# sp-uhh/audio-visual-vad

Measured on AMD Instinct MI355X. Metric: AV frame-pairs/sec (fwd+bwd), higher is better.
Workload: dtype f32; 1 GPU; AV_net fused training step (WaveNet-W0 encoder + ResNet-18 trunk + concat + 2xLSTM1024 + FC, masked BCE, backward, RCCL all-reduce, fused Adam): BASELINE configs[3]/[4] per-GPU shard; per_gpu_frame_pairs=1024, global_frame_pairs=1024, sequences_per_gpu=64, parallelism=dp1, reserved_cus=0, reported_block=median

## Files before the change

audio-visual-vad_amd/csrc/bn_kernels.h:

```cpp
#pragma once
#include "common.h"

constexpr int BN_MAXC = 1024;
constexpr int MAXC = BN_MAXC;
constexpr int STAT_CHUNKS = 512;

template <int MODE>
__global__ void __launch_bounds__(256)
    col_reduce(const float* __restrict__ x, const float* __restrict__ dy, const float* __restrict__ ymask,
               const float* __restrict__ mean, const float* __restrict__ invstd, long M, int C, long rows_per_chunk,
               double* __restrict__ part, const float* __restrict__ msc = nullptr, const float* __restrict__ msh = nullptr,
               const unsigned char* __restrict__ qmask = nullptr) {
  __shared__ double sm[256 * 8];
  const int t = threadIdx.x;
  const int Q = C >> 2, RL = 256 / Q;
  const int q = t % Q, rl = t / Q;
  double s[4] = {0, 0, 0, 0}, ss[4] = {0, 0, 0, 0};
  float mu[4] = {0, 0, 0, 0}, is[4] = {1, 1, 1, 1};
  float ksc[4] = {0, 0, 0, 0}, ksh[4] = {0, 0, 0, 0};
  if (MODE == 1) {
#pragma unroll
    for (int j = 0; j < 4; ++j) { mu[j] = mean[q * 4 + j]; is[j] = invstd[q * 4 + j]; }
    if (msc) {
#pragma unroll
// ... 90 lines not shown
  const int c = blockIdx.x * FIN_CH + (threadIdx.x % FIN_CH);
  if (c >= C || threadIdx.x >= FIN_CH) return;
  float mean, var;
  if (training) {
    const double m = s / (double)M;
    double v = ss / (double)M - m * m;
    if (v < 0) v = 0;
    mean = (float)m; var = (float)v;
    const double unb = M > 1 ? v * (double)M / (double)(M - 1) : v;
    rm[c] = (1.f - momentum) * rm[c] + momentum * mean;
    rv[c] = (1.f - momentum) * rv[c] + momentum * (float)unb;
  } else {
    mean = rm[c]; var = rv[c];
  }
  const float is = 1.0f / sqrtf(var + eps);
  const float sc = gamma[c] * is;
  scale[c] = sc;
  shift[c] = beta[c] - mean * sc;
  mean_o[c] = mean;
  invstd_o[c] = is;
}

__global__ void bn_bwd_finalize(const double* __restrict__ part, int nchunk, long M, int C, const float* __restrict__ gamma,
                                const float* __restrict__ invstd, int training, float* __restrict__ dgamma,
                                float* __restrict__ dbeta, float* __restrict__ coef) {
  double s = 0, ss = 0;
  chunk_sums(part, nchunk, C, s, ss);
  const int c = blockIdx.x * FIN_CH + (threadIdx.x % FIN_CH);
  if (c >= C || threadIdx.x >= FIN_CH) return;
  if (dbeta) dbeta[c] += (float)s;
  if (dgamma) dgamma[c] += (float)ss;
  coef[c] = gamma[c] * invstd[c];
  coef[MAXC + c] = training ? (float)(s / (double)M) : 0.f;
  coef[2 * MAXC + c] = training ? (float)(ss / (double)M) : 0.f;
}

__device__ __forceinline__ float bn_affine(float x, float sc, float sh) { return fmaf(x, sc, sh); }

typedef __bf16 bn_bf16x4 __attribute__((ext_vector_type(4)));
typedef float bn_f32x4 __attribute__((ext_vector_type(4)));
__device__ __forceinline__ void store_quad_bf16(void* base, long quad, const float (&o)[4]) {
  const bn_f32x4 f = {o[0], o[1], o[2], o[3]};
  reinterpret_cast<bn_bf16x4*>(base)[quad] = __builtin_convertvector(f, bn_bf16x4);
}
__device__ __forceinline__ float4 load_quad_bf16(const void* base, long quad) {
  const bn_bf16x4 h = reinterpret_cast<const bn_bf16x4*>(base)[quad];
  const bn_f32x4 f = __builtin_convertvector(h, bn_f32x4);
  return make_float4(f[0], f[1], f[2], f[3]);
}

__device__ __forceinline__ float4 ld4(const float* p, int c) { return *reinterpret_cast<const float4*>(p + c); }

template <bool OB = false, bool IB = false>
__global__ void __launch_bounds__(256)
    bn_act(const float* __restrict__ x, const float* __restrict__ scale, const float* __restrict__ shift,
           const float* __restrict__ idn, const float* __restrict__ iscale, const float* __restrict__ ishift,
           float* __restrict__ y, long nquad, int C, int relu, unsigned char* __restrict__ qmask_out = nullptr) {
  const bool fixed = (256 % (C >> 2)) == 0;
  long i = (long)blockIdx.x * blockDim.x + threadIdx.x;
  int c = (int)((i * 4) % C);
  float4 sc = ld4(scale, c), sh = ld4(shift, c), a = make_float4(0, 0, 0, 0), b = a;
  if (iscale) { a = ld4(iscale, c); b = ld4(ishift, c); }
  for (; i < nquad; i += (long)gridDim.x * blockDim.x) {
    if (!fixed) {
      c = (int)((i * 4) % C);
      sc = ld4(scale, c); sh = ld4(shift, c);
      if (iscale) { a = ld4(iscale, c); b = ld4(ishift, c); }
    }
    const float4 v = reinterpret_cast<const float4*>(x)[i];
    float o[4] = {bn_affine(v.x, sc.x, sh.x), bn_affine(v.y, sc.y, sh.y), bn_affine(v.z, sc.z, sh.z), bn_affine(v.w, sc.w, sh.w)};
    if (idn) {
      const float4 d = IB ? load_quad_bf16(idn, i) : reinterpret_cast<const float4*>(idn)[i];
      if (iscale) {
        o[0] += bn_affine(d.x, a.x, b.x); o[1] += bn_affine(d.y, a.y, b.y);
        o[2] += bn_affine(d.z, a.z, b.z); o[3] += bn_affine(d.w, a.w, b.w);
      } else { o[0] += d.x; o[1] += d.y; o[2] += d.z; o[3] += d.w; }
    }
    if (relu) { o[0] = fmaxf(o[0], 0.f); o[1] = fmaxf(o[1], 0.f); o[2] = fmaxf(o[2], 0.f); o[3] = fmaxf(o[3], 0.f); }
    if constexpr (OB) store_quad_bf16(y, i, o);
    else reinterpret_cast<float4*>(y)[i] = make_float4(o[0], o[1], o[2], o[3]);
    if (qmask_out)
      qmask_out[i] = (unsigned char)((o[0] > 0.f ? 1 : 0) | (o[1] > 0.f ? 2 : 0) | (o[2] > 0.f ? 4 : 0) | (o[3] > 0.f ? 8 : 0));
  }
}

template <bool OB = false>
__global__ void __launch_bounds__(256)
    bn_bwd_apply(const float* __restrict__ x, const float* dy, const float* __restrict__ ymask,
                 const float* __restrict__ mean, const float* __restrict__ invstd, const float* __restrict__ coef,
                 float* dx, float* gout, long nquad, int C, const float* __restrict__ msc = nullptr,
                 const float* __restrict__ msh = nullptr, const unsigned char* __restrict__ qmask = nullptr) {
  const bool fixed = (256 % (C >> 2)) == 0;
  long i = (long)blockIdx.x * blockDim.x + threadIdx.x;
  int c = (int)((i * 4) % C);
  float4 mu = ld4(mean, c), is = ld4(invstd, c), k0 = ld4(coef, c), k1 = ld4(coef + MAXC, c), k2 = ld4(coef + 2 * MAXC, c);
  float4 ms = make_float4(0, 0, 0, 0), mh = ms;
  if (msc) { ms = ld4(msc, c); mh = ld4(msh, c); }
  for (; i < nquad; i += (long)gridDim.x * blockDim.x) {
    if (!fixed) {
      c = (int)((i * 4) % C);
      mu = ld4(mean, c); is = ld4(invstd, c); k0 = ld4(coef, c); k1 = ld4(coef + MAXC, c); k2 = ld4(coef + 2 * MAXC, c);
      if (msc) { ms = ld4(msc, c); mh = ld4(msh, c); }
    }
    const float4 xv = reinterpret_cast<const float4*>(x)[i];
    const float4 d = reinterpret_cast<const float4*>(dy)[i];
    float g[4] = {d.x, d.y, d.z, d.w};
    if (ymask) {
      const float4 y = reinterpret_cast<const float4*>(ymask)[i];
      if (!(y.x > 0.f)) g[0] = 0.f;
      if (!(y.y > 0.f)) g[1] = 0.f;
      if (!(y.z > 0.f)) g[2] = 0.f;
      if (!(y.w > 0.f)) g[3] = 0.f;
    } else if (qmask) {
      const unsigned qm = qmask[i];
      if (!(qm & 1u)) g[0] = 0.f;
      if (!(qm & 2u)) g[1] = 0.f;
      if (!(qm & 4u)) g[2] = 0.f;
      if (!(qm & 8u)) g[3] = 0.f;
    } else if (msc) {
      if (!(fmaf(xv.x, ms.x, mh.x) > 0.f)) g[0] = 0.f;
      if (!(fmaf(xv.y, ms.y, mh.y) > 0.f)) g[1] = 0.f;
      if (!(fmaf(xv.z, ms.z, mh.z) > 0.f)) g[2] = 0.f;
      if (!(fmaf(xv.w, ms.w, mh.w) > 0.f)) g[3] = 0.f;
    }
    const float xs[4] = {xv.x, xv.y, xv.z, xv.w};
    const float m4[4] = {mu.x, mu.y, mu.z, mu.w}, i4[4] = {is.x, is.y, is.z, is.w};
    const float a4[4] = {k0.x, k0.y, k0.z, k0.w}, b4[4] = {k1.x, k1.y, k1.z, k1.w}, c4[4] = {k2.x, k2.y, k2.z, k2.w};
    float o[4];
#pragma unroll
    for (int j = 0; j < 4; ++j) {
      const float xh = (xs[j] - m4[j]) * i4[j];
      o[j] = a4[j] * (g[j] - b4[j] - xh * c4[j]);
    }
    if constexpr (OB) store_quad_bf16(dx, i, o);
    else reinterpret_cast<float4*>(dx)[i] = make_float4(o[0], o[1], o[2], o[3]);
    if (gout) reinterpret_cast<float4*>(gout)[i] = make_float4(g[0], g[1], g[2], g[3]);
  }
}
```

audio-visual-vad_amd/csrc/trunk.hip:

```cpp
#include "bgemm.h"
#include "conv64.h"

using convop::Geom;

namespace {

#include "bn_kernels.h"

constexpr int NCONV = AVVAD_TRUNK_NCONV;

constexpr int NBLOCK = 8;
constexpr int WIDTHS[4] = {64, 128, 256, 512};

struct Block {
  int stage, width;
  int h, w;
  long M;
  bool ds;
  int i1, i2, id;
  size_t in;
  size_t c1, a1;
  size_t c2, cd;
  size_t out, qm;
};
// ... 287 lines not shown
__global__ void __launch_bounds__(256)
    stem_pool_relu_bwd(const float* __restrict__ c0, const float* __restrict__ scale, const float* __restrict__ shift,
                       const unsigned* __restrict__ am, const float* __restrict__ dp0, float* __restrict__ g0,
                       int N, int Hc, int Wc, int Hp, int Wp, const float* __restrict__ mean = nullptr,
                       const float* __restrict__ invstd = nullptr, double* __restrict__ part = nullptr) {
  __shared__ double sm[256 * 8];
  const long total = (long)N * Hc * Wc * 16;
  float s4[4] = {0.f, 0.f, 0.f, 0.f}, q4[4] = {0.f, 0.f, 0.f, 0.f};
  float mu[4] = {0.f, 0.f, 0.f, 0.f}, is[4] = {1.f, 1.f, 1.f, 1.f};
  if (part) {
    const int qc = (int)(((long)blockIdx.x * blockDim.x + threadIdx.x) & 15);
#pragma unroll
    for (int k = 0; k < 4; ++k) { mu[k] = mean[qc * 4 + k]; is[k] = invstd[qc * 4 + k]; }
  }
  for (long i = (long)blockIdx.x * blockDim.x + threadIdx.x; i < total; i += (long)gridDim.x * blockDim.x) {
    const int q = (int)(i & 15);
    long r = i >> 4;
    const int w = (int)(r % Wc); r /= Wc;
    const int h = (int)(r % Hc); const int n = (int)(r / Hc);
    const float4 sc = *reinterpret_cast<const float4*>(scale + q * 4), sh = *reinterpret_cast<const float4*>(shift + q * 4);
    const float4 v = reinterpret_cast<const float4*>(c0)[i];
    const bool pos[4] = {bn_affine(v.x, sc.x, sh.x) > 0.f, bn_affine(v.y, sc.y, sh.y) > 0.f, bn_affine(v.z, sc.z, sh.z) > 0.f,
                         bn_affine(v.w, sc.w, sh.w) > 0.f};
    float g[4] = {0, 0, 0, 0};
    const int ph0 = max(0, h / 2), ph1 = min(Hp - 1, (h + 1) / 2);
    const int pw0 = max(0, w / 2), pw1 = min(Wp - 1, (w + 1) / 2);
    for (int ph = ph0; ph <= ph1; ++ph)
      for (int pw = pw0; pw <= pw1; ++pw) {
        if (h < 2 * ph - 1 || h > 2 * ph + 1 || w < 2 * pw - 1 || w > 2 * pw + 1) continue;
        const unsigned me = (unsigned)((h - (2 * ph - 1)) * 3 + (w - (2 * pw - 1)));
        const long o = ((long)(n * Hp + ph) * Wp + pw) * 16 + q;
        const unsigned a = am[o];
        const float4 dp = reinterpret_cast<const float4*>(dp0)[o];
        if (pos[0] && (a & 255u) == me) g[0] += dp.x;
        if (pos[1] && ((a >> 8) & 255u) == me) g[1] += dp.y;
        if (pos[2] && ((a >> 16) & 255u) == me) g[2] += dp.z;
        if (pos[3] && (a >> 24) == me) g[3] += dp.w;
      }
    reinterpret_cast<float4*>(g0)[i] = make_float4(g[0], g[1], g[2], g[3]);
    if (part) {
      const float xv[4] = {v.x, v.y, v.z, v.w};
#pragma unroll
      for (int k = 0; k < 4; ++k) { s4[k] += g[k]; q4[k] = fmaf(g[k], (xv[k] - mu[k]) * is[k], q4[k]); }
    }
  }
  if (part == nullptr) return;
#pragma unroll
  for (int k = 0; k < 4; ++k) { sm[threadIdx.x * 8 + k] = (double)s4[k]; sm[threadIdx.x * 8 + 4 + k] = (double)q4[k]; }
  __syncthreads();
  if (threadIdx.x < 64) {
    const int c = threadIdx.x, cq = c >> 2, cj = c & 3;
    double a = 0, b = 0;
    for (int l = 0; l < 16; ++l) { a += sm[(l * 16 + cq) * 8 + cj]; b += sm[(l * 16 + cq) * 8 + 4 + cj]; }
    part[((long)blockIdx.x * 2 + 0) * 64 + c] = a;
    part[((long)blockIdx.x * 2 + 1) * 64 + c] = b;
  }
}

template <bool IB = false>
__global__ void avgpool_fwd(const float* __restrict__ y, float* __restrict__ feat, int N, int HW, int C) {
  const long total = (long)N * C;
  for (long i = (long)blockIdx.x * blockDim.x + threadIdx.x; i < total; i += (long)gridDim.x * blockDim.x) {
    const int c = (int)(i % C); const long n = i / C;
    float s = 0.f;
    for (int p = 0; p < HW; ++p) s += IB ? (float)reinterpret_cast<const __bf16*>(y)[(n * HW + p) * C + c] : y[(n * HW + p) * C + c];
    feat[i] = s / (float)HW;
  }
}
__global__ void avgpool_bwd(const float* __restrict__ dfeat, float* __restrict__ dy, int N, int HW, int C) {
  const long total = (long)N * HW * C;
  const float inv = 1.f / (float)HW;
  for (long i = (long)blockIdx.x * blockDim.x + threadIdx.x; i < total; i += (long)gridDim.x * blockDim.x) {
    const int c = (int)(i % C); const long n = i / ((long)HW * C);
    dy[i] = dfeat[n * C + c] * inv;
  }
}
__global__ void zero_f32(float* p, long n) {
  for (long i = (long)blockIdx.x * blockDim.x + threadIdx.x; i < n; i += (long)gridDim.x * blockDim.x) p[i] = 0.f;
}

static inline int ew_grid(long n) { long b = (n + 255) / 256; return (int)(b > 4096 ? 4096 : (b < 1 ? 1 : b)); }

constexpr int STEM_WH = 17;
__global__ void __launch_bounds__(256)
    stem_wgrad_mfma(const float* __restrict__ x, const float* __restrict__ dy, float* __restrict__ slab, int N, int H, int W,
                    int Ho, int Wo, int LDW) {
  extern __shared__ float img[];
  const int lane = threadIdx.x & 63, wave = threadIdx.x >> 6;
  const int li = lane & 31, lh = lane >> 5;
  const int mt = wave >> 1, nt = wave & 1;
  const int tap = mt * 32 + li;
  const int tc = tap < 49 ? tap : 0;
  const int abase = (tc / 7) * LDW + (tc % 7) + 2 * lh;
  const int PH = H + 6, wh = Wo >> 1;
  for (int i = threadIdx.x; i < PH * LDW; i += 256) img[i] = 0.f;
  f32x16 acc;
#pragma unroll
  for (int r = 0; r < 16; ++r) acc[r] = 0.f;
  const int voff = (lh * 64 + nt * 32 + li) * 4;
  for (int n = blockIdx.x; n < N; n += gridDim.x) {
    __syncthreads();
    const float* xn = x + (long)n * H * W;
    for (int i = threadIdx.x; i < H * W; i += 256) {
      const int r = i / W, c = i - r * W;
      img[(r + 3) * LDW + c + 3] = xn[i];
    }
    __syncthreads();
    const __amdgpu_buffer_rsrc_t rdy = brsrc(dy + (long)n * Ho * Wo * 64, Ho * Wo * 64 * 4);
    constexpr int RB = 4;
    float b0[RB][STEM_WH], b1[RB][STEM_WH];
    auto rowload = [&](int ho0, float (&b)[RB][STEM_WH]) {
#pragma unroll
      for (int rr = 0; rr < RB; ++rr)
#pragma unroll
        for (int sw = 0; sw < STEM_WH; ++sw)
          b[rr][sw] = bload(rdy, (sw < wh && ho0 + rr < Ho) ? voff : BUF_OOB, ((ho0 + rr) * Wo + 2 * sw) * 256);
    };
    auto rowmul = [&](int ho0, const float (&b)[RB][STEM_WH]) {
#pragma unroll
      for (int rr = 0; rr < RB; ++rr) {
        if (ho0 + rr >= Ho) break;
        const float* ap = img + abase + 2 * (ho0 + rr) * LDW;
#pragma unroll
        for (int sw = 0; sw < STEM_WH; ++sw)
          if (sw < wh) acc = mfma32(ap[4 * sw], b[rr][sw], acc);
      }
    };
    rowload(0, b0);
    for (int ho = 0; ho < Ho; ho += 2 * RB) {
      if (ho + RB < Ho) rowload(ho + RB, b1);
      __builtin_amdgcn_sched_barrier(0);
      rowmul(ho, b0);
      if (ho + RB >= Ho) break;
      if (ho + 2 * RB < Ho) rowload(ho + 2 * RB, b0);
      __builtin_amdgcn_sched_barrier(0);
      rowmul(ho + RB, b1);
    }
  }
  float* out = slab + (long)blockIdx.x * (49 * 64);
#pragma unroll
  for (int r = 0; r < 16; ++r) {
    const int t = mt * 32 + mfma32_row(r, lh);
    if (t < 49) out[t * 64 + nt * 32 + li] = acc[r];
  }
}
__global__ void __launch_bounds__(256) stem_wgrad_reduce(const float* __restrict__ slab, int nslab, float* __restrict__ pk) {
  __shared__ float sm[8][32];
  const int el = threadIdx.x & 31, grp = threadIdx.x >> 5;
  const int i = blockIdx.x * 32 + el;
  float s = 0.f;
#pragma unroll 4
  for (int b = grp; b < nslab; b += 8) s += slab[(long)b * (49 * 64) + i];
  sm[grp][el] = s;
  __syncthreads();
  if (grp != 0) return;
#pragma unroll
  for (int k = 1; k < 8; ++k) s += sm[k][el];
  pk[i] = s;
}

static inline bool fits_u30(long n) { return n >= 0 && n < (1L << 30); }
static inline bool taps_fit(const Geom& g) { return g.KS * g.KS <= 32; }
static inline bool fits_buf(long n_floats) { return n_floats >= 0 && n_floats < (1L << 29) - 64; }
static inline bool stem_kernel_ok(const Geom& g) {
  const int LDW = (g.W + 6) | 1;
  return g.C == 1 && g.KS == 7 && g.stride == 2 && g.pad == 3 && g.Co == 64 && (size_t)(g.H + 6) * LDW * sizeof(float) <= 48 * 1024 &&
         !avvad_tune().no_stem_kernel;
}
static inline bool stem_wgrad_ok(const Geom& g, bool slab) {
  return stem_kernel_ok(g) && (g.Wo & 1) == 0 && g.Wo <= 2 * STEM_WH && slab && (long)g.Ho * g.Wo * 64 * 4 < (1L << 31);
}
static inline long cls_tile_cap() {
  if (avvad_tune().cls_cap > 0) return avvad_tune().cls_cap;
  return 4L * grid_cus();
}
static inline bool cls_common(const Geom& g, bool slab) {
  return avvad_tune().bf16 == 0 && !avvad_tune().no_cls && slab && g.KS == 3 && g.pad == 1 && g.N >= 128 && g.C % 32 == 0 &&
         g.Co % 32 == 0 && g.Ho >= 2 && g.Wo >= 2 && avvad_tune().igemm_variant < 0 && !avvad_tune().no_buf &&
         avvad_tune().no_streamk == 0;
}
static inline bool conv_fwd_cls_ok(const Geom& g, bool slab) {
  if (!cls_common(g, slab) || g.Co % 4 || g.Co < 128) return false;
  const long tiles = (long)g.Ho * g.Wo * cdiv(g.N, 128) * cdiv(g.Co, 128);
  return tiles <= cls_tile_cap() &&
         fits_buf((long)g.N * g.H * g.W * g.C) && fits_buf(9L * g.C * g.Co);
}
static inline bool conv_dgrad_cls_ok(const Geom& g, bool slab) {
  if (!cls_common(g, slab) || (g.stride != 1 && (g.stride != 2 || avvad_tune().no_s2_cls)) || g.C % 4 || g.C < 128) return false;
  const long tiles = (long)g.H * g.W * cdiv(g.N, 128) * cdiv(g.C, 128);
  return tiles <= cls_tile_cap() &&
         fits_buf((long)g.N * g.Ho * g.Wo * g.Co) && fits_buf(9L * g.C * g.Co);
}
static inline bool conv_wgrad_tap_ok(const Geom& g, bool slab) {
  if (!cls_common(g, slab) || g.C % 128 || g.Co % 4 || g.Co < 128) return false;
  return 9L * (g.C / 128) * cdiv(g.Co, 128) <= cls_tile_cap() &&
         fits_buf((long)g.N * g.H * g.W * g.C) && fits_buf((long)g.N * g.Ho * g.Wo * g.Co);
}
static inline bool conv64_ok(const Geom& g, bool b16) {
  const long M = (long)g.N * g.H * g.W;
  return (b16 || avvad_tune().bf16 == 0) && !avvad_tune().no_conv64 && g.C == 64 && g.Co == 64 && g.KS == 3 && g.stride == 1 &&
         g.pad == 1 && g.Ho == g.H && g.Wo == g.W && M > 0 && fits_buf(M * 64) &&
         (unsigned long)(M + 64) * (unsigned long)(g.H * g.W) < 0x100000000ull;
}
static inline bool conv64_wgrad_ok(const Geom& g, bool slab) {
  return conv64_ok(g, false) && slab && g.W <= conv64::WG_MAXW && (size_t)grid_cus() * conv64::WG_PART <= igemm::SLAB_FLOATS &&
         (long)g.N * g.H * g.W * 256 < (1L << 31);
}

static inline bool native_bf16() { return avvad_tune().bf16 == 1; }
static inline bool bf16_conv_ok(const Geom& g) {
  return g.C % 64 == 0 && g.Co % 64 == 0 && taps_fit(g) && fits_buf((long)g.N * g.H * g.W * g.C / 2) &&
         fits_buf((long)g.N * g.Ho * g.Wo * g.Co / 2) && fits_buf((long)g.KS * g.KS * g.C * g.Co / 2);
}
static inline bool cls16_common(const Geom& g, bool slab) {
  return !avvad_tune().no_cls && slab && g.KS == 3 && g.pad == 1 && g.N >= 128 && g.Ho >= 2 && g.Wo >= 2 && g.Ho * g.Wo <= 9 &&
         avvad_tune().no_streamk == 0;
}
static inline bool conv_fwd16_cls_ok(const Geom& g, bool slab) {
  if (!cls16_common(g, slab) || g.Co < 128) return false;
  return (long)g.Ho * g.Wo * cdiv(g.N, 128) * cdiv(g.Co, 128) <= cls_tile_cap();
}
static inline bool conv_dgrad16_cls_ok(const Geom& g, bool slab) {
  const bool form = g.stride == 1 ? cls16_common(g, slab)
                                  : g.stride == 2 && g.KS == 3 && g.pad == 1 && !avvad_tune().no_cls && !avvad_tune().no_s2_cls &&
                                        avvad_tune().no_streamk == 0 && slab && g.N >= 128;
  return form && g.C >= 128 && (long)g.H * g.W * cdiv(g.N, 128) * cdiv(g.C, 128) <= cls_tile_cap();
}
// ... 192 lines not shown
      const convop::EpiS2 e{dx, g.C, nullptr, 1, 1, g.H, g.W, c.Hc, c.Wc, ph, pw, convop::div_magic(c.Hc * c.Wc), convop::div_magic(c.Wc)};
      if (const int rc = gemm(c, Mc, ntap, e)) return rc;
    }
  return AVVAD_OK;
}
template <bool B16, bool BUF>
static int conv_dgrad_engine(const float* dy, const float* wd, float* dx, const Geom& g, const ConvForm& f, int accumulate, hipStream_t s,
                             float* slab) {
  const int M = g.N * g.H * g.W, T = g.KS * g.KS, K = T * g.Co;
  if constexpr (!B16) {
    if (g.Co % 32 || g.C % 4 || !taps_fit(g)) return AVVAD_EINVAL;
    if (!fits_u30((long)g.N * g.Ho * g.Wo * g.Co) || !fits_u30((long)K * g.C)) return AVVAD_EINVAL;
  }
  const Geom gu = unit_geom<B16>(g, false, true);
  if (f.form == PARITY)
    return dgrad_parity(dx, g, accumulate, s, [&](const convop::S2Class& c, int Mc, int ntap, const convop::EpiS2& e) {
      const int Kc = ntap * g.Co / UNIT<B16>;
      convop::Im2colDgradS2<BUF> a{dy, gu, c, Mc};
      auto b = [&] {
        if constexpr (B16) return bgemm::RowPairsSeg{wd, K / 2, g.C, Kc, T, ntap, {0, 0, 0, 0}, convop::div_magic(ntap)};
        else return convop::ColSegRows<BUF>{wd, g.C, g.C, Kc, ntap, {0, 0, 0, 0}, convop::div_magic(ntap)};
      }();
      for (int ia = 0; ia < c.nkh; ++ia)
        for (int ib = 0; ib < c.nkw; ++ib) {
          const int tap = (c.kh0 + 2 * ia) * g.KS + (c.kw0 + 2 * ib);
          if constexpr (B16) b.tap[ia * c.nkw + ib] = tap;
          else b.rowbase[ia * c.nkw + ib] = tap * g.Co;
        }
      return tile_launch<B16, false>(f, a, b, e, Mc, g.C, Kc, 1, s, slab);
    });
  igemm::EpiStore e{dx, g.C, nullptr, accumulate ? 1 : 0};
  convop::Im2colDgrad<BUF> a{dy, gu, M, convop::tap_div(T, g.KS)};
  const auto b = weight_rows<B16, BUF>(wd, g.C, g.Co, T);
  return tile_launch<B16, true>(f, a, b, e, M, g.C, K / UNIT<B16>, 1, s, slab);
}
static int conv_dgrad(bool b16, const float* dy, const float* wd, float* dx, const Geom& g, int accumulate, hipStream_t s, float* slab) {
  if (b16 && !bf16_conv_ok(g)) return AVVAD_EINVAL;
  const ConvForm f = dgrad_form(g, b16, slab);
  switch (f.form) {
    case CONV64: return conv64_launch(b16, true, dy, wd, dx, g, accumulate, s, nullptr);
    case CLS: return b16 ? conv_dgrad_cls<true>(dy, wd, dx, g, accumulate, s, slab) : conv_dgrad_cls<false>(dy, wd, dx, g, accumulate, s, slab);
    default:
      if (b16) return conv_dgrad_engine<true, true>(dy, wd, dx, g, f, accumulate, s, slab);
      return f.buf ? conv_dgrad_engine<false, true>(dy, wd, dx, g, f, accumulate, s, slab)
                   : conv_dgrad_engine<false, false>(dy, wd, dx, g, f, accumulate, s, slab);
  }
}

template <bool B16>
static int conv_wgrad_tap(const float* x, const float* dy, float* pk, const Geom& g, hipStream_t s, float* slab) {
  const int M = 9 * g.C;
  const igemm::TapSched sc = tap_sched(g, (g.C / 128) * cdiv(g.Co, 128));
  const Geom gu = unit_geom<B16>(g, true, true);
  convop::WgradXTap a{x, gu, M / UNIT<B16>, g.C, g.N, convop::div_magic(gu.C), sc};
  convop::ColDyTap b{dy, gu, gu.Co, g.C, g.N, sc};
  igemm::EpiTap e{pk, g.Co, nullptr, 0};
  e.Mrows = M; e.sched = sc;
  return cls_launch<B16, true>(a, b, e, M, g.Co, s, slab);
}
template <bool B16, bool BUF>
static int conv_wgrad_engine(const float* x, const float* dy, float* pk, const Geom& g, const ConvForm& f, hipStream_t s, float* slab) {
  const int T = g.KS * g.KS, M = T * g.C, K = g.N * g.Ho * g.Wo;
  if (!B16 && g.Co % 4) return AVVAD_EINVAL;
  igemm::ColPlain<4, BUF> b{dy, g.Co / UNIT<B16>, g.Co / UNIT<B16>, K, 0};
  int split = 1;
  if constexpr (!B16) {
    const int ktiles = cdiv(K, igemm::BK);
    if (g.C == 1) {
      igemm::EpiStore e{pk, g.Co, nullptr, 0};
      convop::StemWgradX a{x, g, M, K};
      split = 1024; if (split > ktiles) split = ktiles;
      return igemm::launch<64, 64>(a, b, e, M, g.Co, K, split, s, slab);
    }
    if (g.C % 32) return AVVAD_EINVAL;
    if ((unsigned long)(K + igemm::BK) * (unsigned long)(g.Ho * g.Wo) >= 0x100000000ull) return AVVAD_EINVAL;
    if (!fits_u30((long)g.N * g.H * g.W * g.C) || !fits_u30((long)K * g.Co)) return AVVAD_EINVAL;
    const int nb = cdiv(M, 128) * cdiv(g.Co, f.cols);
    split = cdiv(1024, nb); if (split > ktiles) split = ktiles;
  }
  convop::EpiWgrad e{pk, g.Co, nullptr, 0, 1, g.C, T, convop::div_magic(T), B16 ? 6 : 5};
  convop::WgradX<BUF> a{x, unit_geom<B16>(g, true, false), M / UNIT<B16>, K, convop::div_magic(g.Ho * g.Wo), convop::div_magic(g.Wo)};
  return tile_launch<B16, false, true>(f, a, b, e, M, g.Co, K, split, s, slab);
}
static int conv_wgrad(bool b16, const float* x, const float* dy, float* pk, const Geom& g, hipStream_t s, float* slab) {
  if (b16) {
    const int K = g.N * g.Ho * g.Wo;
    if (!bf16_conv_ok(g)) return AVVAD_EINVAL;
    if ((unsigned long)(K + bgemm::BKU) * (unsigned long)(g.Ho * g.Wo) >= 0x100000000ull) return AVVAD_EINVAL;
  }
  const ConvForm f = wgrad_form(g, b16, slab);
  switch (f.form) {
    case STEM: {
      const int LDW = (g.W + 6) | 1;
      const int nb = g.N < 256 ? g.N : 256;
      hipLaunchKernelGGL(stem_wgrad_mfma, dim3(nb), dim3(256), (size_t)(g.H + 6) * LDW * sizeof(float), s, x, dy, slab, g.N, g.H, g.W,
                         g.Ho, g.Wo, LDW);
      hipLaunchKernelGGL(stem_wgrad_reduce, dim3(49 * 64 / 32), dim3(256), 0, s, slab, nb, pk);
      AVVAD_LAUNCH_CHECK();
      return AVVAD_OK;
    }
    case CONV64: {
      const int NR = g.N * g.H;
      const int grid = NR < grid_cus() ? NR : grid_cus();
      hipLaunchKernelGGL(conv64::wgrad_kernel, dim3(grid), dim3(conv64::WG_WAVES * 64), 0, s, x, dy, slab, NR, g.H, g.W,
                         convop::div_magic((unsigned)g.H));
      hipLaunchKernelGGL(conv64::wgrad_reduce, dim3(conv64::WG_PART / 256), dim3(256), 0, s, (const float*)slab, grid, pk);
      AVVAD_LAUNCH_CHECK();
      return AVVAD_OK;
    }
    case TAP: return b16 ? conv_wgrad_tap<true>(x, dy, pk, g, s, slab) : conv_wgrad_tap<false>(x, dy, pk, g, s, slab);
    default:
      if (b16) return conv_wgrad_engine<true, true>(x, dy, pk, g, f, s, slab);
      return f.buf ? conv_wgrad_engine<false, true>(x, dy, pk, g, f, s, slab) : conv_wgrad_engine<false, false>(x, dy, pk, g, f, s, slab);
  }
}

constexpr const float* NOF = nullptr;
struct BnSlots { float *scale, *shift, *mean, *invstd; };
struct Run {
  const Plan& p;
  float* ws;
  const avvad_trunk_params* prm;
  const avvad_trunk_grads* g;
  const avvad_trunk_desc* d;
  hipStream_t s;
  float* at(size_t off) const { return ws + off; }
  double* part() const { return reinterpret_cast<double*>(ws + p.part); }
  BnSlots bn(int i) const {
    const size_t o = (size_t)i * MAXC;
    return {at(p.bn_scale + o), at(p.bn_shift + o), at(p.bn_mean + o), at(p.bn_invstd + o)};
  }
  long rows(int i) const { const Geom& g = p.geom[i]; return (long)g.N * g.Ho * g.Wo; }
};

struct StatCtx { int nchunk; long rows_per_chunk; };
static StatCtx stat_ctx(long M, int C) {
  const int RL = 256 / (C / 4);
  long per = (M + STAT_CHUNKS - 1) / STAT_CHUNKS;
  if (per < 16L * RL) per = 16L * RL;
  per = (per + RL - 1) / RL * RL;
  return {cdiv(M, per), per};
}

static int fused_chunks(const Run& r, int i, bool b16) {
  if (!r.d->training || avvad_tune().no_fused_stats) return 0;
  const int n = fwd_form(r.p.geom[i], b16, true).chunks;
  return (long)n * r.p.geom[i].Co <= (long)STAT_CHUNKS * MAXC ? n : 0;
}
static int bn_prepare(const Run& r, int i, const float* craw, int fused) {
  const int C = r.p.geom[i].Co;
  const long M = r.rows(i);
  StatCtx sc = stat_ctx(M, C);
  if (fused) {
    sc.nchunk = fused;
  } else if (r.d->training) {
    hipLaunchKernelGGL(col_reduce<0>, dim3(sc.nchunk), dim3(256), 0, r.s, craw, NOF, NOF, NOF, NOF, M, C, sc.rows_per_chunk, r.part());
  }
  const BnSlots bn = r.bn(i);
  hipLaunchKernelGGL(bn_finalize, dim3(cdiv(C, FIN_CH)), dim3(256), 0, r.s, r.part(), sc.nchunk, M, C, r.prm->bn_w[i], r.prm->bn_b[i],
                     r.prm->bn_rm[i], r.prm->bn_rv[i], r.d->training, r.d->momentum, r.d->eps, bn.scale, bn.shift, bn.mean, bn.invstd);
  AVVAD_LAUNCH_CHECK();
  return AVVAD_OK;
}
static int conv_bn(const Run& r, int i, const float* x, float* y) {
  const bool b16 = i > 0 && native_bf16();
  const int fused = fused_chunks(r, i, b16);
  const float* wf = r.at(b16 ? r.p.wf16[i] : r.p.wf[i]);
  if (const int rc = conv_fwd(b16, x, wf, y, r.p.geom[i], r.s, r.at(r.p.slab), fused ? r.part() : nullptr)) return rc;
  return bn_prepare(r, i, y, fused);
}

struct BnBwd {
  bool own_relu = false;
  const float* ymask = nullptr;
  const unsigned char* qmask = nullptr;
  bool out16 = false;
  float* gout = nullptr;
  int reduced_chunks = 0;
};
static int bn_backward(const Run& r, int i, const float* xraw, const float* dy, float* dx, const BnBwd& o) {
  const int C = r.p.geom[i].Co;
  const long M = r.rows(i);
  StatCtx sc = stat_ctx(M, C);
  const BnSlots bn = r.bn(i);
  const float* msc = o.own_relu ? bn.scale : NOF;
  const float* msh = o.own_relu ? bn.shift : NOF;
  const float* ymask = o.own_relu ? NOF : o.ymask;
  const bool qred = o.out16 && o.qmask != nullptr;
  if (o.reduced_chunks > 0)
    sc.nchunk = o.reduced_chunks;
  else
    hipLaunchKernelGGL(col_reduce<1>, dim3(sc.nchunk), dim3(256), 0, r.s, xraw, dy, qred ? NOF : ymask,
                       bn.mean, bn.invstd, M, C, sc.rows_per_chunk, r.part(), msc, msh, qred ? o.qmask : (const unsigned char*)nullptr);
  hipLaunchKernelGGL(bn_bwd_finalize, dim3(cdiv(C, FIN_CH)), dim3(256), 0, r.s, r.part(), sc.nchunk, M, C, r.prm->bn_w[i],
                     bn.invstd, r.d->training, r.g->bn_w[i], r.g->bn_b[i], r.at(r.p.coef));
  const long nq = M * C / 4;
  auto apply = o.out16 ? bn_bwd_apply<true> : bn_bwd_apply<false>;
  hipLaunchKernelGGL(apply, dim3(ew_grid(nq)), dim3(256), 0, r.s, xraw, dy, o.qmask ? NOF : ymask,
                     bn.mean, bn.invstd, r.at(r.p.coef), dx, o.gout, nq, C, msc, msh, o.qmask);
  AVVAD_LAUNCH_CHECK();
  return AVVAD_OK;
}

template <class Tab>
static int tab_shapes(Tab& tab, const Plan& p, int stem_blocks) {
  int nb = 0;
  for (int i = 0; i < NCONV; ++i) {
    const Geom& g = p.geom[i];
    tab.cout[i] = g.Co; tab.cin[i] = g.C; tab.ks[i] = g.KS; tab.blk0[i] = nb;
    nb += i == 0 ? stem_blocks : (g.Co / 32) * (g.C / 32);
  }
  tab.blk0[NCONV] = nb; return nb;
}

}

static bool conv_geom(const avvad_conv_desc* d, Geom* g) {
  if (!d || d->N <= 0 || d->H <= 0 || d->W <= 0 || d->C <= 0 || d->Co <= 0 || d->KS <= 0 || d->stride <= 0 || d->pad < 0)
    return false;
  if (d->H + 2 * d->pad < d->KS || d->W + 2 * d->pad < d->KS) return false;
  const int Ho = (d->H + 2 * d->pad - d->KS) / d->stride + 1, Wo = (d->W + 2 * d->pad - d->KS) / d->stride + 1;
  if (Ho <= 0 || Wo <= 0 || (d->stride != 1 && d->stride != 2)) return false;
  *g = Geom{d->N, d->H, d->W, d->C, Ho, Wo, d->Co, d->KS, d->stride, d->pad};
  return true;
}
extern "C" int avvad_conv2d_pack_weights(const float* w_oihw, float* wf, float* wd, const avvad_conv_desc* d,
                                         avvad_stream_t s) {
  AVVAD_ENTER();
  Geom g;
  if (!w_oihw || !wf || !conv_geom(d, &g)) return AVVAD_EINVAL;
  hipLaunchKernelGGL(pack_weights, dim3(ew_grid((long)g.Co * g.C * g.KS * g.KS)), dim3(256), 0, (hipStream_t)s, w_oihw, wf, wd,
                     g.Co, g.C, g.KS);
  AVVAD_LAUNCH_CHECK();
  return AVVAD_OK;
}
static float* slab_of(void* ws, size_t ws_bytes) { return (ws && ws_bytes >= igemm::SLAB_FLOATS * sizeof(float)) ? (float*)ws : nullptr; }
extern "C" size_t avvad_engine_workspace(void) { return igemm::SLAB_FLOATS * sizeof(float); }
static int conv2d_fwd(bool b16, const void* x, const void* wf, float* y, const avvad_conv_desc* d, void* ws, size_t ws_bytes, avvad_stream_t s) {
  AVVAD_ENTER();
  Geom g;
  if (!x || !wf || !y || !conv_geom(d, &g) || ws_misaligned(ws)) return AVVAD_EINVAL;
  return conv_fwd(b16, (const float*)x, (const float*)wf, y, g, (hipStream_t)s, slab_of(ws, ws_bytes));
}
static int conv2d_dgrad(bool b16, const void* dy, const void* wd, float* dx, const avvad_conv_desc* d, int accumulate, void* ws,
                        size_t ws_bytes, avvad_stream_t s) {
  AVVAD_ENTER();
  Geom g;
  if (!dy || !wd || !dx || !conv_geom(d, &g) || ws_misaligned(ws)) return AVVAD_EINVAL;
  return conv_dgrad(b16, (const float*)dy, (const float*)wd, dx, g, accumulate, (hipStream_t)s, slab_of(ws, ws_bytes));
}
static int conv2d_wgrad(bool b16, const void* x, const void* dy, float* dw_packed, const avvad_conv_desc* d, void* ws, size_t ws_bytes,
                        avvad_stream_t s) {
  AVVAD_ENTER();
  Geom g;
  if (!x || !dy || !dw_packed || !conv_geom(d, &g) || ws_misaligned(ws)) return AVVAD_EINVAL;
  return conv_wgrad(b16, (const float*)x, (const float*)dy, dw_packed, g, (hipStream_t)s, slab_of(ws, ws_bytes));
}
extern "C" int avvad_conv2d_fwd(const float* x, const float* wf, float* y, const avvad_conv_desc* d, void* ws, size_t ws_bytes,
                                avvad_stream_t s) {
  return conv2d_fwd(false, x, wf, y, d, ws, ws_bytes, s);
}
#ifdef AVVAD_PROF
extern "C" int avvad_debug_prof(unsigned long long* out, int reset) {
  if (out) hipMemcpyFromSymbol(out, HIP_SYMBOL(igemm::g_prof), sizeof(unsigned long long) * 8);
  if (reset) { unsigned long long z[8] = {0}; hipMemcpyToSymbol(HIP_SYMBOL(igemm::g_prof), z, sizeof(z)); }
  return 0;
}
extern "C" int avvad_debug_prof_blocks(unsigned long long* out, int n) {
  hipMemcpyFromSymbol(out, HIP_SYMBOL(igemm::g_prof_blk), sizeof(unsigned long long) * 2 * n);
  return 0;
}
extern "C" int avvad_debug_prof_clk(unsigned long long* out, int n) {
  hipMemcpyFromSymbol(out, HIP_SYMBOL(igemm::g_prof_clk), sizeof(unsigned long long) * n);
  return 0;
}
extern "C" int avvad_debug_prof_hw(unsigned long long* out, int n) {
  hipMemcpyFromSymbol(out, HIP_SYMBOL(igemm::g_prof_hw), sizeof(unsigned long long) * n);
  return 0;
}
#endif
extern "C" int avvad_conv2d_dgrad(const float* dy, const float* wd, float* dx, const avvad_conv_desc* d, int accumulate,
                                  void* ws, size_t ws_bytes, avvad_stream_t s) {
// ... 85 lines not shown
  unsigned* am = save ? reinterpret_cast<unsigned*>(r.at(p.am)) : nullptr;
  auto pool = b16 ? stem_bn_relu_pool<true> : stem_bn_relu_pool<false>;
  hipLaunchKernelGGL(pool, dim3(ew_grid((long)d->N * p.h[2] * p.w[2] * 16)), dim3(256), 0, s, r.at(p.c0), bn0.scale, bn0.shift, r.at(p.p0), am,
                     d->N, p.h[1], p.w[1], p.h[2], p.w[2]);
  auto act = b16 ? bn_act<true, false> : bn_act<false, false>;
  auto act_id = b16 ? bn_act<true, true> : bn_act<false, false>;
  for (const Block& k : p.block) {
    const int C = k.width;
    const long nq = k.M * C / 4;
    const float* x = r.at(k.in);
    unsigned char* qmo = save ? reinterpret_cast<unsigned char*>(r.at(k.qm)) : nullptr;
    const BnSlots bn1 = r.bn(k.i1), bn2 = r.bn(k.i2);
    if ((rc = conv_bn(r, k.i1, x, r.at(k.c1)))) return rc;
    hipLaunchKernelGGL(act, dim3(ew_grid(nq)), dim3(256), 0, s, r.at(k.c1), bn1.scale, bn1.shift, NOF, NOF, NOF, r.at(k.a1), nq, C, 1,
                       (unsigned char*)nullptr);
    if ((rc = conv_bn(r, k.i2, r.at(k.a1), r.at(k.c2)))) return rc;
    if (k.ds) {
      if ((rc = conv_bn(r, k.id, x, r.at(k.cd)))) return rc;
      const BnSlots bnd = r.bn(k.id);
      hipLaunchKernelGGL(act, dim3(ew_grid(nq)), dim3(256), 0, s, r.at(k.c2), bn2.scale, bn2.shift, r.at(k.cd), bnd.scale, bnd.shift,
                         r.at(k.out), nq, C, 1, qmo);
    } else {
      hipLaunchKernelGGL(act_id, dim3(ew_grid(nq)), dim3(256), 0, s, r.at(k.c2), bn2.scale, bn2.shift, x, NOF, NOF, r.at(k.out), nq, C, 1, qmo);
    }
  }
  const Block& last = p.block[NBLOCK - 1];
  auto avg = b16 ? avgpool_fwd<true> : avgpool_fwd<false>;
  hipLaunchKernelGGL(avg, dim3(ew_grid((long)d->N * last.width)), dim3(256), 0, s, r.at(last.out), feat, d->N, last.h * last.w, last.width);
  AVVAD_LAUNCH_CHECK();
  return AVVAD_OK;
}

extern "C" int avvad_trunk_bwd(const float* frames, const avvad_trunk_params* prm, const float* dfeat,
                               const avvad_trunk_grads* g, const avvad_trunk_desc* d, void* wsv, size_t ws_bytes,
                               avvad_stream_t sv) {
  AVVAD_ENTER();
  BwdCuCap cu_cap;
  if (!frames || !prm || !dfeat || !g || !wsv || ws_misaligned(wsv) || !trunk_desc_ok(d) || !d->save_for_backward) return AVVAD_EINVAL;
  const Plan p = make_plan(d);
  if (ws_bytes < p.total * sizeof(float)) return AVVAD_EWORKSPACE;
  const Run r{p, (float*)wsv, prm, g, d, (hipStream_t)sv};
  hipStream_t s = r.s; int rc;
  float *G0 = r.at(p.G[0]), *G1 = r.at(p.G[1]), *G2 = r.at(p.G[2]), *G3 = r.at(p.G[3]);
  const Block& last = p.block[NBLOCK - 1];
  hipLaunchKernelGGL(avgpool_bwd, dim3(ew_grid(last.M * last.width)), dim3(256), 0, s, dfeat, G0, d->N, last.h * last.w, last.width);
  const bool b16 = native_bf16();
  const size_t* wd = b16 ? p.wd16 : p.wd;
  auto wgrad = [&](int i, const float* x, const float* dy) {
    return g->conv_w[i] ? conv_wgrad(i > 0 && b16, x, dy, r.at(p.wg[i]), p.geom[i], s, r.at(p.slab)) : AVVAD_OK;
  };
  auto dgrad = [&](int i, const float* dy, float* dx, int acc) { return conv_dgrad(b16, dy, r.at(wd[i]), dx, p.geom[i], acc, s, r.at(p.slab)); };
  for (int kb = NBLOCK - 1; kb >= 0; --kb) {
    const Block& k = p.block[kb];
    const float* x = r.at(k.in);
    BnBwd under_out, under_own;
    under_out.ymask = r.at(k.out);
    under_out.qmask = reinterpret_cast<const unsigned char*>(r.at(k.qm));
    under_out.out16 = under_own.out16 = b16; under_own.own_relu = true;
    if (k.ds) {
      if ((rc = bn_backward(r, k.i2, r.at(k.c2), G0, G1, under_out))) return rc;
      if ((rc = bn_backward(r, k.id, r.at(k.cd), G0, G2, under_out))) return rc;
      if ((rc = wgrad(k.id, x, G2))) return rc;
      if ((rc = dgrad(k.id, G2, G3, 0))) return rc;
    } else {
      under_out.gout = G3;
      if ((rc = bn_backward(r, k.i2, r.at(k.c2), G0, G1, under_out))) return rc;
    }
    if ((rc = wgrad(k.i2, r.at(k.a1), G1))) return rc;
    if ((rc = dgrad(k.i2, G1, G2, 0))) return rc;
    if ((rc = bn_backward(r, k.i1, r.at(k.c1), G2, G1, under_own))) return rc;
    if ((rc = wgrad(k.i1, x, G1))) return rc;
    if ((rc = dgrad(k.i1, G1, G3, 1))) return rc;
    float* t = G0; G0 = G3; G3 = t;
  }
  if (g->conv_w[0] || g->bn_w[0] || g->bn_b[0]) {
    float* g0 = r.at(p.g0);
    const BnSlots bn0 = r.bn(0);
    const bool fuse0 = !avvad_tune().no_fused_stats;
    int grid0 = ew_grid((long)d->N * p.h[1] * p.w[1] * 16);
    if (fuse0 && grid0 > 2048) grid0 = 2048;
    hipLaunchKernelGGL(stem_pool_relu_bwd, dim3(grid0), dim3(256), 0, s, r.at(p.c0), bn0.scale, bn0.shift,
                       reinterpret_cast<const unsigned*>(r.at(p.am)), G0, g0, d->N, p.h[1], p.w[1], p.h[2], p.w[2],
                       fuse0 ? bn0.mean : NOF, fuse0 ? bn0.invstd : NOF, fuse0 ? r.part() : (double*)nullptr);
    BnBwd stem; stem.reduced_chunks = fuse0 ? grid0 : 0;
    if ((rc = bn_backward(r, 0, r.at(p.c0), g0, g0, stem))) return rc;
    if ((rc = wgrad(0, frames, g0))) return rc;
  }
  UnpackTab tab;
  const int nb = tab_shapes(tab, p, cdiv(64 * 3 * 49, 256));
  bool any = false;
  for (int i = 0; i < NCONV; ++i) {
    tab.pk[i] = r.at(p.wg[i]);
    tab.dw[i] = g->conv_w[i];
    any = any || g->conv_w[i];
  }
  if (any) hipLaunchKernelGGL(unpack_all, dim3(nb), dim3(256), 0, s, tab);
  AVVAD_LAUNCH_CHECK();
  return AVVAD_OK;
}
```

Before: 60550 frame-pairs/s.

## Fuse stem BN backward apply into stem weight-gradient MFMA kernel

For the stem conv, the BN backward apply pass (computing dx from raw conv output, upstream grad and BN coefficients) is skipped when fused stats are on. The dx computation is instead done inline in stem_wgrad_mfma, which now loads both dy and the raw conv output and applies the BN formula before the MFMA. This removes one full elementwise read/write pass over the stem activation. In exchange the wgrad kernel does twice the global loads and uses more registers. The double-buffer scheme becomes a single-buffer loop with a take() step, which may reduce load/compute overlap.

```diff
diff --git a/audio-visual-vad_amd/csrc/bn_kernels.h b/audio-visual-vad_amd/csrc/bn_kernels.h
--- a/audio-visual-vad_amd/csrc/bn_kernels.h
+++ b/audio-visual-vad_amd/csrc/bn_kernels.h
@@ -196,6 +196,17 @@
     if (qmask_out)
       qmask_out[i] = (unsigned char)((o[0] > 0.f ? 1 : 0) | (o[1] > 0.f ? 2 : 0) | (o[2] > 0.f ? 4 : 0) | (o[3] > 0.f ? 8 : 0));
   }
+}
+
+struct BnDx { float mu, is, k0, k1, k2; };
+__device__ __forceinline__ float bn_bwd_dx(float x, float g, const BnDx& k) {
+#pragma clang fp contract(off)
+  const float xh = (x - k.mu) * k.is;
+  return k.k0 * fmaf(-xh, k.k2, g - k.k1);
+}
+struct BnDxSrc { const float *x, *mean, *invstd, *coef; };
+__device__ __forceinline__ BnDx bn_dx_consts(const BnDxSrc& s, int c) {
+  return {s.mean[c], s.invstd[c], s.coef[c], s.coef[MAXC + c], s.coef[2 * MAXC + c]};
 }
 
 template <bool OB = false>
@@ -242,10 +253,7 @@
     const float a4[4] = {k0.x, k0.y, k0.z, k0.w}, b4[4] = {k1.x, k1.y, k1.z, k1.w}, c4[4] = {k2.x, k2.y, k2.z, k2.w};
     float o[4];
 #pragma unroll
-    for (int j = 0; j < 4; ++j) {
-      const float xh = (xs[j] - m4[j]) * i4[j];
-      o[j] = a4[j] * (g[j] - b4[j] - xh * c4[j]);
-    }
+    for (int j = 0; j < 4; ++j) o[j] = bn_bwd_dx(xs[j], g[j], BnDx{m4[j], i4[j], a4[j], b4[j], c4[j]});
     if constexpr (OB) store_quad_bf16(dx, i, o);
     else reinterpret_cast<float4*>(dx)[i] = make_float4(o[0], o[1], o[2], o[3]);
     if (gout) reinterpret_cast<float4*>(gout)[i] = make_float4(g[0], g[1], g[2], g[3]);
diff --git a/audio-visual-vad_amd/csrc/trunk.hip b/audio-visual-vad_amd/csrc/trunk.hip
--- a/audio-visual-vad_amd/csrc/trunk.hip
+++ b/audio-visual-vad_amd/csrc/trunk.hip
@@ -393,67 +393,63 @@
 static inline int ew_grid(long n) { long b = (n + 255) / 256; return (int)(b > 4096 ? 4096 : (b < 1 ? 1 : b)); }
 
 constexpr int STEM_WH = 17;
+template <bool BN>
 __global__ void __launch_bounds__(256)
     stem_wgrad_mfma(const float* __restrict__ x, const float* __restrict__ dy, float* __restrict__ slab, int N, int H, int W,
-                    int Ho, int Wo, int LDW) {
+                    int Ho, int Wo, int LDW, BnDxSrc bn) {
   extern __shared__ float img[];
-  const int lane = threadIdx.x & 63, wave = threadIdx.x >> 6;
-  const int li = lane & 31, lh = lane >> 5;
-  const int mt = wave >> 1, nt = wave & 1;
-  const int tap = mt * 32 + li;
-  const int tc = tap < 49 ? tap : 0;
-  const int abase = (tc / 7) * LDW + (tc % 7) + 2 * lh;
-  const int PH = H + 6, wh = Wo >> 1;
+  const int lane = threadIdx.x & 63, wave = threadIdx.x >> 6, li = lane & 31, lh = lane >> 5, mt = wave >> 1, nt = wave & 1;
+  const int tap = mt * 32 + li, tc = tap < 49 ? tap : 0;
+  const int abase = (tc / 7) * LDW + (tc % 7) + 2 * lh, PH = H + 6, wh = Wo >> 1;
   for (int i = threadIdx.x; i < PH * LDW; i += 256) img[i] = 0.f;
-  f32x16 acc;
-#pragma unroll
-  for (int r = 0; r < 16; ++r) acc[r] = 0.f;
+  f32x16 acc = {};
   const int voff = (lh * 64 + nt * 32 + li) * 4;
+  const BnDx k = BN ? bn_dx_consts(bn, nt * 32 + li) : BnDx{};
   for (int n = blockIdx.x; n < N; n += gridDim.x) {
     __syncthreads();
     const float* xn = x + (long)n * H * W;
-    for (int i = threadIdx.x; i < H * W; i += 256) {
-      const int r = i / W, c = i - r * W;
-      img[(r + 3) * LDW + c + 3] = xn[i];
-    }
+    for (int i = threadIdx.x; i < H * W; i += 256) img[(i / W + 3) * LDW + i % W + 3] = xn[i];
     __syncthreads();
     const __amdgpu_buffer_rsrc_t rdy = brsrc(dy + (long)n * Ho * Wo * 64, Ho * Wo * 64 * 4);
-    constexpr int RB = 4;
-    float b0[RB][STEM_WH], b1[RB][STEM_WH];
-    auto rowload = [&](int ho0, float (&b)[RB][STEM_WH]) {
+    const __amdgpu_buffer_rsrc_t rc0 = brsrc((BN ? bn.x : dy) + (long)n * Ho * Wo * 64, Ho * Wo * 64 * 4);
+    constexpr int RB = 4, NB = RB * STEM_WH;
+    float ld[NB], lc[BN ? NB : 1], cur[NB];
+    auto rowload = [&](int ho0) {
 #pragma unroll
       for (int rr = 0; rr < RB; ++rr)
 #pragma unroll
-        for (int sw = 0; sw < STEM_WH; ++sw)
-          b[rr][sw] = bload(rdy, (sw < wh && ho0 + rr < Ho) ? voff : BUF_OOB, ((ho0 + rr) * Wo + 2 * sw) * 256);
+        for (int sw = 0; sw < STEM_WH; ++sw) {
+          const int vo = (sw < wh && ho0 + rr < Ho) ? voff : BUF_OOB, so = ((ho0 + rr) * Wo + 2 * sw) * 256;
+          ld[rr * STEM_WH + sw] = bload(rdy, vo, so); if constexpr (BN) lc[rr * STEM_WH + sw] = bload(rc0, vo, so);
+        }
     };
-    auto rowmul = [&](int ho0, const float (&b)[RB][STEM_WH]) {
+    auto take = [&]() {
+#pragma unroll
+      for (int e = 0; e < NB; ++e) { if constexpr (BN) cur[e] = bn_bwd_dx(lc[e], ld[e], k); else cur[e] = ld[e]; }
+    };
+    auto rowmul = [&](int ho0) {
 #pragma unroll
       for (int rr = 0; rr < RB; ++rr) {
         if (ho0 + rr >= Ho) break;
         const float* ap = img + abase + 2 * (ho0 + rr) * LDW;
 #pragma unroll
         for (int sw = 0; sw < STEM_WH; ++sw)
-          if (sw < wh) acc = mfma32(ap[4 * sw], b[rr][sw], acc);
+          if (sw < wh) acc = mfma32(ap[4 * sw], cur[rr * STEM_WH + sw], acc);
       }
     };
-    rowload(0, b0);
-    for (int ho = 0; ho < Ho; ho += 2 * RB) {
-      if (ho + RB < Ho) rowload(ho + RB, b1);
+    rowload(0);
+    for (int ho = 0; ho < Ho; ho += RB) {
+      take();
+      if (ho + RB < Ho) rowload(ho + RB);
       __builtin_amdgcn_sched_barrier(0);
-      rowmul(ho, b0);
-      if (ho + RB >= Ho) break;
-      if (ho + 2 * RB < Ho) rowload(ho + 2 * RB, b0);
+      rowmul(ho);
       __builtin_amdgcn_sched_barrier(0);
-      rowmul(ho + RB, b1);
     }
   }
   float* out = slab + (long)blockIdx.x * (49 * 64);
 #pragma unroll
-  for (int r = 0; r < 16; ++r) {
-    const int t = mt * 32 + mfma32_row(r, lh);
-    if (t < 49) out[t * 64 + nt * 32 + li] = acc[r];
-  }
+  for (int r = 0; r < 16; ++r)
+    if (const int t = mt * 32 + mfma32_row(r, lh); t < 49) out[t * 64 + nt * 32 + li] = acc[r];
 }
 __global__ void __launch_bounds__(256) stem_wgrad_reduce(const float* __restrict__ slab, int nslab, float* __restrict__ pk) {
   __shared__ float sm[8][32];
@@ -812,7 +808,7 @@
   convop::WgradX<BUF> a{x, unit_geom<B16>(g, true, false), M / UNIT<B16>, K, convop::div_magic(g.Ho * g.Wo), convop::div_magic(g.Wo)};
   return tile_launch<B16, false, true>(f, a, b, e, M, g.Co, K, split, s, slab);
 }
-static int conv_wgrad(bool b16, const float* x, const float* dy, float* pk, const Geom& g, hipStream_t s, float* slab) {
+static int conv_wgrad(bool b16, const float* x, const float* dy, float* pk, const Geom& g, hipStream_t s, float* slab, const BnDxSrc* bn = nullptr) {
   if (b16) {
     const int K = g.N * g.Ho * g.Wo;
     if (!bf16_conv_ok(g)) return AVVAD_EINVAL;
@@ -823,8 +819,8 @@
     case STEM: {
       const int LDW = (g.W + 6) | 1;
       const int nb = g.N < 256 ? g.N : 256;
-      hipLaunchKernelGGL(stem_wgrad_mfma, dim3(nb), dim3(256), (size_t)(g.H + 6) * LDW * sizeof(float), s, x, dy, slab, g.N, g.H, g.W,
-                         g.Ho, g.Wo, LDW);
+      hipLaunchKernelGGL(bn ? stem_wgrad_mfma<true> : stem_wgrad_mfma<false>, dim3(nb), dim3(256), (size_t)(g.H + 6) * LDW * sizeof(float), s,
+                         x, dy, slab, g.N, g.H, g.W, g.Ho, g.Wo, LDW, bn ? *bn : BnDxSrc{});
       hipLaunchKernelGGL(stem_wgrad_reduce, dim3(49 * 64 / 32), dim3(256), 0, s, slab, nb, pk);
       AVVAD_LAUNCH_CHECK();
       return AVVAD_OK;
@@ -907,6 +903,7 @@
   bool out16 = false;
   float* gout = nullptr;
   int reduced_chunks = 0;
+  bool coef_only = false;
 };
 static int bn_backward(const Run& r, int i, const float* xraw, const float* dy, float* dx, const BnBwd& o) {
   const int C = r.p.geom[i].Co;
@@ -925,9 +922,9 @@
   hipLaunchKernelGGL(bn_bwd_finalize, dim3(cdiv(C, FIN_CH)), dim3(256), 0, r.s, r.part(), sc.nchunk, M, C, r.prm->bn_w[i],
                      bn.invstd, r.d->training, r.g->bn_w[i], r.g->bn_b[i], r.at(r.p.coef));
   const long nq = M * C / 4;
-  auto apply = o.out16 ? bn_bwd_apply<true> : bn_bwd_apply<false>;
-  hipLaunchKernelGGL(apply, dim3(ew_grid(nq)), dim3(256), 0, r.s, xraw, dy, o.qmask ? NOF : ymask,
-                     bn.mean, bn.invstd, r.at(r.p.coef), dx, o.gout, nq, C, msc, msh, o.qmask);
+  if (!o.coef_only)
+    hipLaunchKernelGGL(o.out16 ? bn_bwd_apply<true> : bn_bwd_apply<false>, dim3(ew_grid(nq)), dim3(256), 0, r.s, xraw, dy, o.qmask ? NOF : ymask,
+                       bn.mean, bn.invstd, r.at(r.p.coef), dx, o.gout, nq, C, msc, msh, o.qmask);
   AVVAD_LAUNCH_CHECK();
   return AVVAD_OK;
 }
@@ -1179,9 +1176,11 @@
     hipLaunchKernelGGL(stem_pool_relu_bwd, dim3(grid0), dim3(256), 0, s, r.at(p.c0), bn0.scale, bn0.shift,
                        reinterpret_cast<const unsigned*>(r.at(p.am)), G0, g0, d->N, p.h[1], p.w[1], p.h[2], p.w[2],
                        fuse0 ? bn0.mean : NOF, fuse0 ? bn0.invstd : NOF, fuse0 ? r.part() : (double*)nullptr);
-    BnBwd stem; stem.reduced_chunks = fuse0 ? grid0 : 0;
+    const bool in_wgrad = fuse0 && g->conv_w[0] && wgrad_form(p.geom[0], false, true).form == STEM;
+    BnBwd stem; stem.reduced_chunks = fuse0 ? grid0 : 0; stem.coef_only = in_wgrad;
     if ((rc = bn_backward(r, 0, r.at(p.c0), g0, g0, stem))) return rc;
-    if ((rc = wgrad(0, frames, g0))) return rc;
+    const BnDxSrc bn{r.at(p.c0), bn0.mean, bn0.invstd, r.at(p.coef)};
+    if (g->conv_w[0] && (rc = conv_wgrad(false, frames, g0, r.at(p.wg[0]), p.geom[0], s, r.at(p.slab), in_wgrad ? &bn : nullptr))) return rc;
   }
   UnpackTab tab;
   const int nb = tab_shapes(tab, p, cdiv(64 * 3 * 49, 256));
```

Result: no change. 60730 frame-pairs/s (median of 6 runs) (+0.3%).
